# spaceandtimefdn/blitzar

Hardware: NVIDIA H100
Metric: MSM throughput (scalar*point terms/sec), ristretto255, n=2^20 per GPU (higher is better)
Workload: dtype u32 limbs (integer modular arithmetic)

## Files before the change

### blitzar_b200/api.py

```python
import ctypes as C
import os

import numpy as np

_HERE = os.path.dirname(os.path.abspath(__file__))
LIB_PATH = os.path.join(_HERE, "lib", "libblitzar_b200.so")

SXT_CPU_BACKEND, SXT_GPU_BACKEND = 1, 2
SXT_CURVE_RISTRETTO255, SXT_CURVE_BLS_381, SXT_CURVE_BN_254, SXT_CURVE_GRUMPKIN = 0, 1, 2, 3
CURVE_SIZES = {0: (160, 160, 32), 1: (144, 104, 48), 2: (96, 72, 72), 3: (96, 72, 72)}
COMPACT_BYTES = {0: 120, 1: 96, 2: 64, 3: 64}

SXT_SYMBOLS = [
    "sxt_init", "sxt_curve25519_compute_pedersen_commitments",
    "sxt_curve25519_compute_pedersen_commitments_with_generators",
    "sxt_bls12_381_g1_compute_pedersen_commitments_with_generators",
    "sxt_bn254_g1_uncompressed_compute_pedersen_commitments_with_generators",
    "sxt_grumpkin_uncompressed_compute_pedersen_commitments_with_generators",
    "sxt_ristretto255_get_generators", "sxt_curve25519_get_one_commit",
    "sxt_curve25519_prove_inner_product", "sxt_curve25519_verify_inner_product",
    "sxt_multiexp_handle_new", "sxt_multiexp_handle_new_from_file",
    "sxt_multiexp_handle_write_to_file", "sxt_multiexp_handle_free",
    "sxt_fixed_multiexponentiation", "sxt_fixed_packed_multiexponentiation",
    "sxt_fixed_vlen_multiexponentiation", "sxt_prove_sumcheck",
]
B200_SYMBOLS = [
    "b200_set_device", "b200_launch_count", "b200_point_bytes", "b200_malloc", "b200_free",
    "b200_memcpy_h2d", "b200_memcpy_d2h", "b200_synchronize", "b200_event_create",
    "b200_event_record", "b200_event_elapsed_ms", "b200_event_destroy", "b200_commit_device",
    "b200_combine_partials_device", "b200_fixed_msm_device",
    "b200_combine_partials_projective_device", "b200_set_tuning", "b200_profile_accumulate",
    "b200_profile_read", "b200_set_reduce_groups", "b200_stream",
    "b200_synthetic_generators_device", "b200_commit_host_partials",
    "b200_fixed_msm_host_partials", "b200_multiexp_handle_new_device",
    "b200_selftest_lane_arithmetic", "b200_selftest_sort", "b200_partition_table_device",
    "b200_multiexp_handle_write_partition_table",
    "b200_compute_pedersen_commitments_with_offsets", "b200_commit_device_with_offsets",
    "b200_multiexp_handle_add_partition_table", "b200_multiexp_handle_partition_window",
]


class sxt_config(C.Structure):
    _fields_ = [("backend", C.c_int), ("num_precomputed_generators", C.c_uint64)]


class sxt_sequence_descriptor(C.Structure):
    _fields_ = [("element_nbytes", C.c_uint8), ("n", C.c_uint64), ("data", C.c_void_p),
                ("is_signed", C.c_int)]


_lib = None


def lib():
    global _lib
    if _lib is None:
        if not os.path.exists(LIB_PATH):
            raise RuntimeError(f"{LIB_PATH} is missing: run `python -m blitzar_b200.build` "
                               "(blitzar_b200 has no CPU fallback)")
        L = C.CDLL(LIB_PATH)
        L.sxt_init.restype = C.c_int
        L.sxt_ristretto255_get_generators.restype = C.c_int
        L.sxt_curve25519_get_one_commit.restype = C.c_int
        L.sxt_multiexp_handle_new.restype = C.c_void_p
        L.sxt_multiexp_handle_new_from_file.restype = C.c_void_p
        L.b200_launch_count.restype = C.c_ulonglong
        L.b200_point_bytes.restype = C.c_uint
        L.b200_malloc.restype = C.c_void_p
        L.b200_multiexp_handle_new_device.restype = C.c_void_p
        L.b200_event_create.restype = C.c_void_p
        L.b200_stream.restype = C.c_void_p
        L.b200_event_elapsed_ms.restype = C.c_float
        _lib = L
    return _lib


_initialized = False


def sxt_init(backend=SXT_GPU_BACKEND, num_precomputed_generators=0, device=None):
    global _initialized
    if _initialized:
        return 0
    if device is not None:
        lib().b200_set_device(C.c_int(device))
    cfg = sxt_config(backend, num_precomputed_generators)
    rc = lib().sxt_init(C.byref(cfg))
    if rc == 0:
        _initialized = True
    return rc

# ... 170 lines not shown
    def record(self):
        lib().b200_event_record(C.c_void_p(self.e))

    def elapsed_ms(self, stop):
        return float(lib().b200_event_elapsed_ms(C.c_void_p(self.e), C.c_void_p(stop.e)))


def commit_device(curve_id, columns_shape, scalar_ptrs, generators_ptr, out_commit_ptr=None,
                  out_partial_ptr=None, offset_generators=0):
    num = len(columns_shape)
    arr = (sxt_sequence_descriptor * max(1, num))()
    for i, (n, nbytes, is_signed) in enumerate(columns_shape):
        arr[i].element_nbytes = nbytes
        arr[i].n = n
        arr[i].data = scalar_ptrs[i]
        arr[i].is_signed = int(is_signed)
    lib().b200_commit_device(C.c_uint(curve_id), C.c_void_p(out_commit_ptr),
                             C.c_void_p(out_partial_ptr), C.c_uint32(num), arr,
                             C.c_void_p(generators_ptr), C.c_uint64(offset_generators))


def commit_device_with_offsets(curve_id, columns_shape, scalar_ptrs, generators_ptr, offsets,
                               out_commit_ptr=None, out_partial_ptr=None):
    num = len(columns_shape)
    arr = (sxt_sequence_descriptor * max(1, num))()
    for i, (n, nbytes, is_signed) in enumerate(columns_shape):
        arr[i].element_nbytes = nbytes
        arr[i].n = n
        arr[i].data = scalar_ptrs[i]
        arr[i].is_signed = int(is_signed)
    offsets = _offsets(offsets, num)
    lib().b200_commit_device_with_offsets(C.c_uint(curve_id), C.c_void_p(out_commit_ptr),
                                          C.c_void_p(out_partial_ptr), C.c_uint32(num), arr,
                                          C.c_void_p(generators_ptr), _ptr(offsets))


def selftest_lane_arithmetic(warps=64, seed=1):
    lib().b200_selftest_lane_arithmetic.restype = C.c_uint
    return int(lib().b200_selftest_lane_arithmetic(C.c_uint(warps), C.c_uint(seed)))


def selftest_sort(columns_shape, scalar_ptrs, window_bits=0):
    num = len(columns_shape)
    arr = (sxt_sequence_descriptor * max(1, num))()
    for i, (n, nbytes, is_signed) in enumerate(columns_shape):
        arr[i].element_nbytes = nbytes
        arr[i].n = n
        arr[i].data = scalar_ptrs[i]
        arr[i].is_signed = int(is_signed)
    lib().b200_selftest_sort.restype = C.c_uint
    return int(lib().b200_selftest_sort(arr, C.c_uint(num), C.c_uint(window_bits)))


def synthetic_generators_device(curve_id, out_ptr, n, first=0, projective=False):
    lib().b200_synthetic_generators_device(C.c_uint(curve_id), C.c_void_p(out_ptr), C.c_uint64(n),
                                           C.c_uint64(first), C.c_int(1 if projective else 0))


def partition_table_bytes(curve_id, n, window_width):
    return -(-n // window_width) * (COMPACT_BYTES[curve_id] << window_width)


def partition_table_device(curve_id, out_ptr, gens_ptr, n, window_width=0):
    lib().b200_partition_table_device(C.c_uint(curve_id), C.c_void_p(out_ptr), C.c_void_p(gens_ptr),
                                      C.c_uint64(n), C.c_uint(window_width))


def synthetic_generators(curve_id, n, first=0, projective=False):
    stride = CURVE_SIZES[curve_id][0 if (projective or curve_id == 0) else 1]
    buf = DeviceBuffer(n * stride)
    synthetic_generators_device(curve_id, buf.ptr, n, first, projective)
    out = buf.to_host((n, stride))
    buf.free()
    return out


def commit_host_partials(curve_id, columns, generators, out_partial_ptr, offset_generators=0):
    desc, keep = make_descriptors(columns)
    lib().b200_commit_host_partials(C.c_uint(curve_id), C.c_void_p(out_partial_ptr),
                                    C.c_uint32(len(columns)), desc, _ptr(generators),
                                    C.c_uint64(offset_generators))


def fixed_msm_device(handle, out_res_ptr, out_partial_ptr, element_num_bytes, num_outputs, n,
                     scalars_ptr):
    lib().b200_fixed_msm_device(C.c_void_p(out_res_ptr), C.c_void_p(out_partial_ptr),
                                C.c_void_p(handle.h), C.c_int(0), C.c_uint(element_num_bytes),
                                None, None, C.c_uint(num_outputs), C.c_uint(n),
                                C.c_void_p(scalars_ptr))


def fixed_msm_host_partials(handle, out_partial_ptr, element_num_bytes, num_outputs, n, scalars):
    lib().b200_fixed_msm_host_partials(C.c_void_p(out_partial_ptr), C.c_void_p(handle.h),
                                       C.c_int(0), C.c_uint(element_num_bytes), None, None,
                                       C.c_uint(num_outputs), C.c_uint(n), _ptr(scalars))


def combine_partials_projective_device(curve_id, out_ptr, partials_ptr, num_parts, count):
    lib().b200_combine_partials_projective_device(C.c_uint(curve_id), C.c_void_p(out_ptr),
                                                  C.c_void_p(partials_ptr), C.c_uint32(num_parts),
                                                  C.c_uint32(count))


def synchronize():
    lib().b200_synchronize()

# ... 63 lines not shown
```

### blitzar_b200/csrc/api.cu

```cuda
#include <algorithm>
#include <cctype>
#include <cstdint>
#include <cstdio>
#include <cstdlib>
#include <cstring>
#include <condition_variable>
#include <functional>
#include <mutex>
#include <thread>
#include <memory>
#include <string>
#include <vector>

#include "engine_api.cuh"

using namespace b200;

namespace {

struct State {
  bool initialized = false;
  int device = -1;
  cudaStream_t stream = nullptr;
  cudaStream_t copy_stream = nullptr;
// ... 1296 lines not shown
    }
    if (i >= 1) {
      const int k = (int)((i - 1) & 1);
      B200_CUDA(cudaEventSynchronize(copied[k]));
      B200_REQUIRE(std::fwrite(host[k], chunk_size(i - 1), 1, f) == 1, "short write");
    }
  }
  B200_REQUIRE(std::fclose(f) == 0, "short write");
  stream_sync(s);
  for (int k = 0; k < 2; ++k) {
    if (host[k])
      B200_CUDA(cudaFreeHost(host[k]));
    B200_CUDA(cudaEventDestroy(built[k]));
    B200_CUDA(cudaEventDestroy(copied[k]));
  }
}
unsigned b200_multiexp_handle_add_partition_table(struct sxt_multiexp_handle* handle,
                                                  unsigned window_width) {
  std::lock_guard<std::mutex> lock(g_mutex);
  require_init("b200_multiexp_handle_add_partition_table");
  HandleSet* hs = reinterpret_cast<HandleSet*>(handle);
  B200_REQUIRE(hs != nullptr, "null handle");
  return handle_add_partition_table(hs, window_width);
}
unsigned b200_multiexp_handle_partition_window(const struct sxt_multiexp_handle* handle) {
  std::lock_guard<std::mutex> lock(g_mutex);
  const HandleSet* hs = reinterpret_cast<const HandleSet*>(handle);
  B200_REQUIRE(hs != nullptr, "null handle");
  return hs->shards.empty() ? 0u : hs->shards[0]->ptable_w;
}
unsigned b200_selftest_lane_arithmetic(unsigned warps, unsigned seed) {
  std::lock_guard<std::mutex> lock(g_mutex);
  require_init("b200_selftest_lane_arithmetic");
  return selftest_lane_arithmetic(ctx(), warps, seed);
}
unsigned b200_selftest_sort(const sxt_sequence_descriptor* columns, unsigned num,
                            unsigned window_bits) {
  std::lock_guard<std::mutex> lock(g_mutex);
  require_init("b200_selftest_sort");
  B200_REQUIRE(num == 0 || columns != nullptr, "columns == nullptr");
  B200_REQUIRE(window_bits <= 20, "window_bits in 0..20");
  return selftest_sort(ctx(), columns, num, window_bits);
}
void b200_set_reduce_groups(unsigned g1, unsigned gn) {
  std::lock_guard<std::mutex> lock(g_mutex);
  auto pow2 = [](unsigned v, unsigned dflt) {
    if (v < 2)
      return dflt;
    unsigned p = 2;
    while (p * 2 <= v)
      p *= 2;
    return p;
  };
  g_state.opt.reduce_g1 = pow2(g1, 16u);
  g_state.opt.reduce_gn = pow2(gn, 4u);
}
void b200_profile_accumulate(int enable) {
  std::lock_guard<std::mutex> lock(g_mutex);
  KernelTimer::get().enabled = enable != 0;
}
void b200_profile_read(float* total_ms, unsigned* launches) {
  std::lock_guard<std::mutex> lock(g_mutex);
  KernelTimer::get().read(total_ms, launches);
}
void b200_set_tuning(unsigned window_bits, unsigned chunk1, unsigned chunkn) {
  std::lock_guard<std::mutex> lock(g_mutex);
  g_state.opt.window_bits = window_bits;
  g_state.opt.chunk1 = chunk1;
  g_state.opt.chunkn = chunkn ? chunkn : 8;
}

}
```

### blitzar_b200/csrc/engine.cuh

```cuda
#pragma once
#include <cstdint>
#include <vector>

#include "engine_api.cuh"
#include "msm.cuh"
#include "partition_msm.cuh"
#include "ptable.cuh"
#include "synth.cuh"

namespace b200 {

inline uint64_t check_descriptors(const sxt_sequence_descriptor* d, uint32_t num) {
  B200_REQUIRE(d != nullptr, "descriptors == nullptr");
  uint64_t longest = 0;
  for (uint32_t i = 0; i < num; ++i) {
    B200_REQUIRE(d[i].n == 0 || d[i].data != nullptr, "descriptor.n > 0 with data == nullptr");
    B200_REQUIRE(d[i].element_nbytes != 0 && d[i].element_nbytes <= 32,
                 "descriptor.element_nbytes must be in 1..32");
    if (d[i].is_signed)
      B200_REQUIRE(d[i].element_nbytes <= 16 &&
                       (d[i].element_nbytes & (d[i].element_nbytes - 1)) == 0,
                   "signed columns need a power-of-two element_nbytes <= 16");
    B200_REQUIRE(d[i].n < (1ull << 31), "column too long");
    longest = longest < d[i].n ? d[i].n : longest;
// ... 364 lines not shown
        cost_t += (double)col.n * (col.bit_width / table_c + 1) + 2.5 * nb_t;
        cost_v += (double)(col.bit_width / cv + 1) * ((double)col.n + 2.5 * nb_v);
      }
    return cost_t < cost_v;
  }
  static std::vector<u32> partition_route(const EngineCtx& ctx, const Handle* h,
                                          const std::vector<ColumnDesc>& cols) {
    std::vector<u32> routed;
    if (!h->ptable || ctx.partition_policy == 2)
      return routed;
    const double kLookup = 1.0, kDouble = 300.0;
    const bool table_mode = prefer_table(cols, h->window_bits, h->windows, ctx.opt);
    u64 max_n = 0;
    u32 max_width = 1, ncols = 0;
    for (auto& col : cols)
      if (col.n) {
        max_n = std::max<u64>(max_n, col.n);
        max_width = std::max(max_width, col.bit_width);
        ++ncols;
      }
    if (ncols == 0)
      return routed;
    const u32 cv = ctx.opt.window_bits ? ctx.opt.window_bits
                                       : choose_window_bits(max_n, max_width, ncols, sizeof(Point));
    const double nb_v = (double)(1u << (cv - 1)), w = h->ptable_w;
    for (u32 j = 0; j < (u32)cols.size(); ++j) {
      const ColumnDesc& col = cols[j];
      if (col.n == 0)
        continue;
      const double n = col.n, b = col.bit_width;
      const double engine =
          table_mode ? n * (double)(col.bit_width / h->window_bits + 1) +
                           2.5 * (double)(1u << (h->window_bits - 1))
                     : (double)(col.bit_width / cv + 1) * (n + 2.5 * nb_v);
      const double table = kLookup * b * std::ceil(n / w) + kDouble * b;
      if (ctx.partition_policy == 1 || table < engine)
        routed.push_back(j);
    }
    return routed;
  }
  static void synth_generators(const EngineCtx& ctx, void* out_dev, uint64_t n, uint64_t first,
                               bool projective) {
    Synth<C>::generators(ctx.s, out_dev, n, first, projective);
  }
  static void partition_table(const EngineCtx& ctx, const void* gens, uint64_t n, unsigned w,
                              uint64_t first_group, uint64_t groups, void* out_dev) {
    build_partition_table<C>(ctx.s, (const Gen*)gens, n, w, first_group, groups,
                             (unsigned char*)out_dev);
  }
  static void partition_gens(const EngineCtx& ctx, const void* gens, uint64_t n, unsigned w,
                             uint64_t first_group, uint64_t groups, void* out_gens) {
    build_partition_table<C>(ctx.s, (const Gen*)gens, n, w, first_group, groups, (Gen*)out_gens);
  }
};

#define B200_DEFINE_CURVE_VTABLE(NAME, C)                                                          \
  const CurveVTable NAME = {C::kCurveId,                                                           \
                            (unsigned)sizeof(typename C::Point),                                   \
                            (unsigned)sizeof(typename C::Gen),                                     \
                            (unsigned)C::kAbiGenBytes,                                             \
                            (unsigned)C::kAbiProjBytes,                                            \
                            (unsigned)C::kAbiCommitBytes,                                          \
                            &CurveOps<C>::commit_device,                                           \
                            &CurveOps<C>::commit_device_offsets,                                   \
                            &CurveOps<C>::fixed_device,                                            \
                            &CurveOps<C>::ingest_projective,                                       \
                            &CurveOps<C>::gens_to_projective,                                      \
                            &CurveOps<C>::store,                                                   \
                            &CurveOps<C>::sum_parts,                                               \
                            &CurveOps<C>::synth_generators,                                        \
                            (unsigned)C::kAbiCompactBytes,                                         \
                            &CurveOps<C>::ingest_compact_table,                                    \
                            &CurveOps<C>::build_table,                                             \
                            &CurveOps<C>::partition_table,                                         \
                            &CurveOps<C>::partition_gens}

}
```

### blitzar_b200/csrc/engine_api.cuh

```cuda
#pragma once
#include <algorithm>
#include <cmath>
#include <cstdint>
#include <vector>

#include "../../include/blitzar_b200.h"
#include "runtime.cuh"

namespace b200 {

struct MsmOptions {
  u32 window_bits = 0;
  u32 chunk1 = 0;
  u32 chunkn = 8;
  u32 reduce_g1 = 16;
  u32 reduce_gn = 4;
  u64 quad_threshold = 32768;
  u64 max_group_entries = 1ull << 30;
  u64 max_range_entries = 1ull << 31;
  int pair_levels = -1;
  u32 pair_batch = 0;
  int range_skew = 0;
  u32 uniform_add = 2;
  u32 gens_normalized = 0;
  const u32* unit_veto = nullptr;
  u32 normalize_gens = 1;
  u32 lane_tail = 1;
  u32 scatter_window_major = 0;
  u32 sort_path = 1;
  u32 table_policy = 0;
};

struct EngineCtx {
  stream_t s;
  MsmOptions opt;
  const void* builtin;
  uint64_t num_builtin;
  stream_t tail = stream_t();
  u32 builtin_window_bits = 0, builtin_windows = 0;
  u32 partition_policy = 0;
};

struct Handle {
  unsigned curve_id;
  unsigned n;
  void* gens;
  unsigned window_bits = 0, windows = 1;
  void* ptable = nullptr;
  unsigned ptable_w = 0;
  uint64_t ptable_groups = 0;
};

inline unsigned table_window_bits(uint64_t n, size_t gen_bytes, double budget_bytes) {
  if (n < 1024)
    return 0;
  unsigned best = 0;
  double best_cost = 1e300;
  for (unsigned c = 10; c <= 20; ++c) {
    const double W = 256 / c + 1;
    if (W * (double)n * (double)gen_bytes > budget_bytes || W * (double)n >= 2147483648.0)
      continue;
    const double cost = W * (double)n + 2.5 * (double)(1u << (c - 1));
    if (cost < best_cost) {
      best_cost = cost;
      best = c;
    }
  }
  return best;
// ... 69 lines not shown
      if (n_[j] > b)
        iv.push_back({base[j] + b, base[j] + std::min(e, n_[j])});
    std::sort(iv.begin(), iv.end());
    std::vector<Piece> out;
    size_t k = 0;
    for (auto& v : iv) {
      while (segments[k].pos + segments[k].count <= v.first)
        ++k;
      const Piece& s = segments[k];
      if (!out.empty() && out.back().pos + out.back().count >= v.first && out.back().pos >= s.pos) {
        out.back().count = std::max(out.back().count, v.second - out.back().pos);
        continue;
      }
      out.push_back({s.src + (v.first - s.pos), v.first, v.second - v.first});
    }
    return out;
  }

private:
  std::vector<uint64_t> n_;
  static uint64_t offset(const uint64_t* offsets, uint32_t j) { return offsets ? offsets[j] : 0; }
};

struct CurveVTable {
  unsigned curve_id, point_bytes, gen_bytes, abi_gen_bytes, abi_proj_bytes, abi_commit_bytes;
  void (*commit_device)(const EngineCtx&, void* out_commitments, void* out_partials, uint32_t num,
                        const sxt_sequence_descriptor* d, const void* generators_dev,
                        uint64_t offset_generators, uint32_t num_ranges, range_wait_fn wait,
                        void* wait_user);
  void (*commit_device_offsets)(const EngineCtx&, void* out_commitments, void* out_partials,
                                uint32_t num, const sxt_sequence_descriptor* d,
                                const void* generators_dev, const uint64_t* offsets, bool packed,
                                uint32_t num_ranges, range_wait_fn wait, void* wait_user);
  void (*fixed_device)(const EngineCtx&, void* out_res, void* out_partials, const Handle* h,
                       int mode, unsigned element_num_bytes, const unsigned* bit_table,
                       const unsigned* lengths, unsigned num_outputs, unsigned n,
                       const uint8_t* scalars_dev);
  void (*ingest_projective)(const EngineCtx&, const void* raw_dev, void* gens, uint64_t n);
  void (*gens_to_projective)(const EngineCtx&, const void* gens, void* out_dev, uint64_t n);
  void (*store)(const EngineCtx&, const void* pts, void* out_dev, uint64_t count, bool commit);
  void (*sum_parts)(const EngineCtx&, const void* parts, uint32_t nparts, uint32_t count,
                    void* out_pts);
  void (*synth_generators)(const EngineCtx&, void* out_dev, uint64_t n, uint64_t first,
                           bool projective);
  unsigned abi_compact_bytes;
  void (*ingest_compact_table)(const EngineCtx&, const void* table_dev, unsigned window_width,
                               void* gens, uint64_t n);
  void (*build_table)(const EngineCtx&, void* table, uint64_t n, unsigned window_bits,
                      unsigned windows);
  void (*partition_table)(const EngineCtx&, const void* gens, uint64_t n, unsigned w,
                          uint64_t first_group, uint64_t groups, void* out_dev);
  void (*partition_gens)(const EngineCtx&, const void* gens, uint64_t n, unsigned w,
                         uint64_t first_group, uint64_t groups, void* out_gens);
};
extern const CurveVTable kVTableEd25519, kVTableBls12381, kVTableBn254, kVTableGrumpkin;

inline const CurveVTable& curve_vtable(unsigned curve_id) {
  switch (curve_id) {
  case SXT_CURVE_RISTRETTO255:
    return kVTableEd25519;
  case SXT_CURVE_BLS_381:
    return kVTableBls12381;
  case SXT_CURVE_BN_254:
    return kVTableBn254;
  case SXT_CURVE_GRUMPKIN:
    return kVTableGrumpkin;
  default:
    die("unsupported curve id", __FILE__, __LINE__);
  }
}

void ipa_prove(const EngineCtx& ctx, uint8_t* l_vector, uint8_t* r_vector, uint8_t* ap_value,
               uint8_t* transcript203, uint64_t n, uint64_t generators_offset,
               const uint8_t* a_vector, const uint8_t* b_vector);
int ipa_verify(const EngineCtx& ctx, uint8_t* transcript203, uint64_t n,
               uint64_t generators_offset, const uint8_t* b_vector, const uint8_t* product,
               const uint8_t* a_commit160, const uint8_t* l_vector, const uint8_t* r_vector,
               const uint8_t* ap_value);

unsigned selftest_lane_arithmetic(const EngineCtx& ctx, unsigned warps, unsigned seed);
unsigned selftest_sort(const EngineCtx& ctx, const sxt_sequence_descriptor* d, unsigned num,
                       unsigned window_bits);

void launch_builtin_generators(const EngineCtx& ctx, void* gens, uint64_t first, uint64_t n);

}
```

### blitzar_b200/csrc/msm.cuh

```cuda
#pragma once
#include <algorithm>
#include <vector>

#include "batch_affine.cuh"
#include "curve.cuh"
#include "engine_api.cuh"
#include "lanefield.cuh"

namespace b200 {

struct ColumnDesc {
  const unsigned char* base;
  u64 row_stride;
  u32 bit_offset;
  u32 bit_width;
  u32 n;
  u32 is_signed;
  u32 first_window;
  u32 num_windows;
  u32 table_n;
  u32 gen_base;
};
B200_HD u32 bucket_windows(const ColumnDesc& col) { return col.table_n ? (col.num_windows ? 1u : 0u) : col.num_windows; }

// ... 690 lines not shown
            out_pieces[2 * t] = acc;
          }
          first_seg = false;
          cur = k;
          fetch(acc, i, true);
        }
      }
    }
    if (final_level) {
      put_bucket(cur, acc, writer);
      return;
    }
    if (!writer)
      return;
    if (first_seg) {
      out_keys[2 * t] = cur;
      out_pieces[2 * t] = acc;
      out_keys[2 * t + 1] = cur;
      out_pieces[2 * t + 1] = C::identity();
    } else {
      out_keys[2 * t + 1] = cur;
      out_pieces[2 * t + 1] = acc;
    }
  }
};

struct WindowUsedBody {
  static constexpr int kBlock = 64;
  const u32* bucket_end;
  u32 nbuckets;
  u32* window_used;
  B200_HD void operator()(u64 w) const {
    u32 lo = w ? bucket_end[w * nbuckets - 1] : 0u;
    u32 hi = bucket_end[(w + 1) * nbuckets - 1];
    if (hi != lo)
      window_used[w] = 1u;
  }
};

struct WindowUsedFromCountsBody {
  static constexpr int kBlock = 128;
  const u32* counts;
  u64 nkeys;
  u32 nbuckets;
  u32* window_used;
  B200_HD void operator()(u64 t) const {
    const u64 b = t * 256, e = b + 256 < nkeys ? b + 256 : nkeys;
    for (u64 k = b; k < e; ++k)
      if (counts[k])
        window_used[k / nbuckets] = 1u;
  }
};

template <class C, class Ex = SeqExec> struct ReduceBody {
  static constexpr int kBlock = 64;
  typedef typename C::Point Point;
  const Point* X;
  const Point* Cin;
  u32 m_in, g, log2g;
  Point* Xout;
  Point* Cout;
  const u32* window_used;
  u32 nbuckets;
  B200_HD void operator()(u64 tid) const {
    const u64 t = tid / Ex::kLanes;
    const bool writer = (tid % Ex::kLanes) == 0;
    const u32 m_out = m_in / g;
    const u32 w = (u32)(t / m_out), k = (u32)(t % m_out);
    if (window_used[w] == 0) {
      if (writer) {
        Xout[t] = C::identity();
        Cout[t] = C::identity();
      }
      return;
    }
    const Point* x = X + (u64)w * m_in + (u64)k * g;
    Point run = x[g - 1];
    Point acc = Cin ? C::identity() : run;
    if (Cin) {
      acc = run;
      if (g == 1)
        acc = C::identity();
    }
    for (u32 r = g - 1; r-- > 0;) {
      C::template add<Ex>(run, run, x[r]);
      if (r > 0 || !Cin)
        C::template add<Ex>(acc, acc, run);
    }
    if (Cin) {
      const Point* cin = Cin + (u64)w * m_in + (u64)k * g;
      for (u32 r = 0; r < g; ++r)
        C::template add<Ex>(acc, acc, cin[r]);
    }
    for (u32 i = 0; i < log2g; ++i)
      C::template dbl<Ex>(run, run);
    if (writer) {
      Xout[t] = run;
      Cout[t] = acc;
    }
  }
};

template <class C, class X = SeqExec> struct CombineBody {
  static constexpr int kBlock = 32;
  typedef typename C::Point Point;
  const Point* S;
  const ColumnDesc* cols;
  u32 c;
  Point* out;
  B200_HD void operator()(u64 tid) const {
    const u64 j = tid / X::kLanes;
    const bool writer = (tid % X::kLanes) == 0;
    const ColumnDesc col = cols[j];
    if (col.num_windows == 0 || col.n == 0) {
      if (writer)
        out[j] = C::identity();
      return;
    }
    const u32 nw = bucket_windows(col);
    Point acc = S[col.first_window + nw - 1];
    for (u32 w = nw - 1; w-- > 0;) {
      for (u32 i = 0; i < c; ++i)
        C::template dbl<X>(acc, acc);
      C::template add<X>(acc, acc, S[col.first_window + w]);
    }
    if (writer)
      out[j] = acc;
  }
};

#if defined(__CUDACC__) && !defined(B200_EMULATE)
#define B200_LANE_TAIL 1
struct CombineLaneBody {
  static constexpr int kBlock = 32;
  typedef Ed25519 C;
  const C::Point* S;
  const ColumnDesc* cols;
  u32 c;
  C::Point* out;
  __device__ void operator()(u64 tid) const {
    const u64 j = tid >> 5;
    const ColumnDesc col = cols[j];
    if (col.num_windows == 0 || col.n == 0) {
      if ((tid & 31u) == 0)
        out[j] = C::identity();
      return;
    }
    const lane10::Lane L = lane10::lane_info();
    const u32 nw = bucket_windows(col);
    C::Point acc = S[col.first_window + nw - 1];
    for (u32 w = nw - 1; w-- > 0;) {
      u32 t;
      const u32 v = lane10::dbl_n(L, lane10::slice_point(L, acc), (int)c, t);
      lane10::gather_point(acc, v, t);
// ... 646 lines not shown
                          u32* d_window_used, const MsmOptions& opt, stream_t tail,
                          RangeHook* hook = nullptr) {
  const StagedRange r(s, plan, begin, end);
  if (r.total_terms == 0)
    return;
  gens += begin;
  StageRange nvtx_sort("msm: digit count + scan + scatter");
  const u64 max_entries = r.max_entries, nkeys = plan.nkeys;
  u32 L = 0;
  if constexpr (C::kBatchAffine) {
    const double mean = (double)max_entries / (double)nkeys;
    if (opt.pair_levels >= 0)
      L = (u32)opt.pair_levels;
    else if (max_entries >= (1ull << 23))
      while (L < 6 && (double)(32u << L) <= mean)
        ++L;
    while (L > 0 && max_entries + nkeys * ((1ull << L) - 1) >= (1ull << 32) - (1ull << L))
      --L;
  }
  const SortedLayout sorted = sort_entries(s, plan, r, L, opt, d_window_used);
  B200_LOG(3, "range [%llu, %llu): %llu terms, %llu entries max, c=%u, %llu keys, pair levels %u",
           (unsigned long long)begin, (unsigned long long)end, (unsigned long long)r.total_terms,
           (unsigned long long)max_entries, plan.c, (unsigned long long)nkeys, L);
  WalkInput<C> walk{gens, sorted.entries, sorted.d_m, max_entries};
  std::vector<void*> to_free;
  if (hook)
    hook->before_accumulate();
  KernelTimer::get().begin(s);
  StageRange nvtx_acc("msm: bucket accumulation");
  if constexpr (C::kBatchAffine) {
    if (L) {
      walk = run_pair_levels<C>(s, L, sorted.entries, gens, sorted.d_m, sorted.slots_max,
                                opt.pair_batch);
      to_free = {(void*)walk.gens, (void*)walk.entries};
    }
  }
  typedef typename C::Point Point;
  Point* target = add_into ? (Point*)dev_alloc(nkeys * sizeof(Point), s) : d_buckets;
  const bool unit = walk.gens == gens && opt.gens_normalized;
  const stream_t cs =
      chunk_walk<C>(s, tail, walk, sorted.d_m, unit, opt.unit_veto, target, opt, to_free);
  if (add_into) {
    launch(MergeBucketsBody<C>{sorted.counts, sorted.starts, target, d_buckets}, nkeys, cs);
    dev_free(target, cs);
  }
  to_free.insert(to_free.end(), {sorted.d_m, sorted.counts, sorted.starts});
  for (void* ptr : to_free)
    dev_free(ptr, cs);
  dev_free(sorted.entries, s);
  dev_free((void*)r.d_cols, s);
}

template <class C>
void msm_finish(stream_t s, const MsmPlan& plan, const typename C::Point* d_buckets,
                const u32* d_window_used, typename C::Point* out, const MsmOptions& opt) {
  typedef typename C::Point Point;
  StageRange nvtx_fin("msm: bucket reduction + window combination");
  const u32 total_windows = plan.total_windows, nbuckets = plan.nbuckets, ncols = plan.ncols;
  ColumnDesc* d_cols =
      (ColumnDesc*)stage_to_device(s, plan.cols.data(), ncols * sizeof(ColumnDesc));
  Point* d_S = nullptr;
  u32 m = nbuckets;
  const Point* X = d_buckets;
  const Point* Cin = nullptr;
  std::vector<void*> to_free;
  if (m == 1) {
    d_S = (Point*)dev_alloc(total_windows * sizeof(Point), s);
    copy_d2d(d_S, d_buckets, total_windows * sizeof(Point), s);
  }
  bool first = true;
  while (m > 1) {
    u32 g = first ? std::min<u32>(opt.reduce_g1, m) : std::min<u32>(opt.reduce_gn, m);
    u32 log2g = 0;
    while ((1u << log2g) < g)
      ++log2g;
    u32 m_out = m / g;
    Point* Xout = (Point*)dev_alloc((u64)total_windows * m_out * sizeof(Point), s);
    Point* Cout = (Point*)dev_alloc((u64)total_windows * m_out * sizeof(Point), s);
    if ((u64)total_windows * m_out <= opt.quad_threshold)
      launch(ReduceBody<C, QuadExecConv>{X, Cin, m, g, log2g, Xout, Cout, d_window_used, nbuckets},
             (u64)total_windows * m_out * QuadExec::kLanes, s);
    else
      launch(ReduceBody<C>{X, Cin, m, g, log2g, Xout, Cout, d_window_used, nbuckets},
             (u64)total_windows * m_out, s);
    to_free.push_back(Xout);
    if (m_out > 1)
      to_free.push_back(Cout);
    X = Xout;
    Cin = Cout;
    m = m_out;
    first = false;
    if (m == 1)
      d_S = Cout;
  }
  for (void* ptr : to_free)
    dev_free(ptr, s);
  bool uniform_windows = true;
  for (u32 j = 1; j < ncols; ++j)
    uniform_windows = uniform_windows && bucket_windows(plan.cols[j]) == bucket_windows(plan.cols[0]);
#ifdef B200_LANE_TAIL
  bool lane_done = false;
  if constexpr (C::kCurveId == kRistretto255) {
    if (ncols <= 2048 && opt.lane_tail) {
      launch(CombineLaneBody{d_S, d_cols, plan.c, out}, (u64)ncols * 32, s);
      lane_done = true;
    }
  }
  if (lane_done) {
  } else
#endif
  if (ncols <= opt.quad_threshold && uniform_windows)
    launch(CombineBody<C, QuadExecConv>{d_S, d_cols, plan.c, out}, (u64)ncols * QuadExec::kLanes,
           s);
  else if (ncols <= opt.quad_threshold)
    launch(CombineBody<C, QuadExec>{d_S, d_cols, plan.c, out}, (u64)ncols * QuadExec::kLanes, s);
  else
    launch(CombineBody<C>{d_S, d_cols, plan.c, out}, ncols, s);
  dev_free(d_S, s);
  dev_free(d_cols, s);
}

template <class C>
void msm_run(stream_t s, const typename C::Gen* gens, std::vector<ColumnDesc> cols,
             typename C::Point* out, const MsmOptions& opt = MsmOptions(), u32 num_ranges = 1,
             RangeHook* hook = nullptr, stream_t tail = stream_t()) {
  typedef typename C::Point Point;
  if (cols.empty())
    return;
  MsmPlan plan = msm_make_plan(std::move(cols), opt, sizeof(Point));
  B200_LOG(2, "msm: curve %u, %u columns, longest %llu, %llu terms, window %u bits, %u bucket sets%s",
           C::kCurveId, plan.ncols, (unsigned long long)plan.max_n,
           (unsigned long long)plan.total_terms, plan.c, plan.total_windows,
           plan.ncols && plan.cols[0].table_n ? " (fixed-base table)" : "");
  if (plan.total_terms == 0 || plan.total_windows == 0) {
    if (hook)
      hook->before_range(0, plan.max_n);
    fill_identity<C>(s, out, plan.ncols);
    return;
  }
  Point* d_buckets = (Point*)dev_alloc(plan.nkeys * sizeof(Point), s);
  fill_identity<C>(s, d_buckets, plan.nkeys);
  u32* d_window_used = (u32*)dev_alloc(plan.total_windows * sizeof(u32), s);
  dev_zero(d_window_used, plan.total_windows * sizeof(u32), s);
  if (num_ranges < 1)
    num_ranges = 1;
  const u64 limit = opt.max_range_entries ? opt.max_range_entries : (1ull << 31);
  const u64 needed = (plan.total_entries + limit - 1) / limit;
  if (needed > num_ranges)
    num_ranges = (u32)std::min<u64>(needed, plan.max_n);
// ... 18 lines not shown
```

### include/blitzar_b200.h

```cpp
#ifndef BLITZAR_B200_H
#define BLITZAR_B200_H

#include <stdint.h>

#ifdef __cplusplus
extern "C" {
#endif

#define SXT_CPU_BACKEND 1
#define SXT_GPU_BACKEND 2
#define SXT_CURVE_RISTRETTO255 0
#define SXT_CURVE_BLS_381 1
#define SXT_CURVE_BN_254 2
#define SXT_CURVE_GRUMPKIN 3
#define SXT_FIELD_SCALAR255 0
#define SXT_FIELD_GRUMPKIN 1

struct sxt_config { int backend; uint64_t num_precomputed_generators; };
struct sxt_ristretto255_compressed { uint8_t ristretto_bytes[32]; };
struct sxt_bls12_381_g1_compressed { uint8_t g1_bytes[48]; };
struct sxt_curve25519_scalar { uint8_t bytes[32]; };
struct sxt_transcript { uint8_t bytes[203]; };
struct sxt_ristretto255 { uint64_t X[5]; uint64_t Y[5]; uint64_t Z[5]; uint64_t T[5]; };
struct sxt_bls12_381_g1 { uint64_t X[6]; uint64_t Y[6]; };
// ... 94 lines not shown
void* b200_stream(void);
void* b200_event_create(void);
void b200_event_record(void* event);
float b200_event_elapsed_ms(void* start, void* stop);
void b200_event_destroy(void* event);

void b200_commit_device(unsigned curve_id, void* out_commitments, void* out_partials,
                        uint32_t num_sequences, const struct sxt_sequence_descriptor* descriptors,
                        const void* generators, uint64_t offset_generators);
void b200_commit_host_partials(unsigned curve_id, void* out_partials, uint32_t num_sequences,
                               const struct sxt_sequence_descriptor* descriptors,
                               const void* generators, uint64_t offset_generators);
void b200_compute_pedersen_commitments_with_offsets(unsigned curve_id, void* commitments,
                                                    uint32_t num_sequences,
                                                    const struct sxt_sequence_descriptor* descriptors,
                                                    const void* generators, const uint64_t* offsets);
void b200_commit_device_with_offsets(unsigned curve_id, void* out_commitments, void* out_partials,
                                     uint32_t num_sequences,
                                     const struct sxt_sequence_descriptor* descriptors,
                                     const void* generators, const uint64_t* offsets);
void b200_fixed_msm_host_partials(void* out_partials, const struct sxt_multiexp_handle* handle,
                                  int mode, unsigned element_num_bytes,
                                  const unsigned* output_bit_table, const unsigned* output_lengths,
                                  unsigned num_outputs, unsigned n, const uint8_t* scalars);
struct sxt_multiexp_handle* b200_multiexp_handle_new_device(unsigned curve_id,
                                                            const void* generators_dev,
                                                            unsigned n);
void b200_combine_partials_device(unsigned curve_id, void* out_commitments, const void* partials,
                                  uint32_t num_parts, uint32_t count);
void b200_fixed_msm_device(void* out_res, void* out_partials,
                           const struct sxt_multiexp_handle* handle, int mode,
                           unsigned element_num_bytes, const unsigned* output_bit_table,
                           const unsigned* output_lengths, unsigned num_outputs, unsigned n,
                           const uint8_t* scalars);
void b200_combine_partials_projective_device(unsigned curve_id, void* out_res,
                                             const void* partials, uint32_t num_parts,
                                             uint32_t count);
void b200_synthetic_generators_device(unsigned curve_id, void* out_generators, uint64_t n,
                                      uint64_t first, int projective);
void b200_partition_table_device(unsigned curve_id, void* out_table_dev, const void* generators_dev,
                                 uint64_t n, unsigned window_width);
void b200_multiexp_handle_write_partition_table(const struct sxt_multiexp_handle* handle,
                                                const char* filename, unsigned window_width);
unsigned b200_multiexp_handle_add_partition_table(struct sxt_multiexp_handle* handle,
                                                  unsigned window_width);
unsigned b200_multiexp_handle_partition_window(const struct sxt_multiexp_handle* handle);
unsigned b200_selftest_lane_arithmetic(unsigned warps, unsigned seed);
unsigned b200_selftest_sort(const struct sxt_sequence_descriptor* columns, unsigned num,
                            unsigned window_bits);
void b200_profile_accumulate(int enable);
void b200_profile_read(float* total_ms, unsigned* launches);
void b200_set_tuning(unsigned window_bits, unsigned chunk1, unsigned chunkn);
void b200_set_reduce_groups(unsigned g1, unsigned gn);

#ifdef __cplusplus
}
#endif
#endif
```

Before: 336.3 million.

## Replace multi-level bucket reduction with segment pass plus block-level shared-memory fold

Bucket reduction used to run as a chain of global-memory levels, each with a fixed group size. It now runs as an adaptive first segment pass, then a ReduceFoldBody kernel that folds many segment partials per block in shared memory with a tree of adds and doublings. The goal is fewer kernel launches and global round trips, plus better occupancy, during the reduction stage. A selftest compares the new path against the old one. The default reduce_g1 changes to 0 so the segment length is picked automatically.

Result: no change. 338.4 million (median of 6 runs) (+0.6%).

```diff
diff --git a/blitzar_b200/api.py b/blitzar_b200/api.py
--- a/blitzar_b200/api.py
+++ b/blitzar_b200/api.py
@@ -37,6 +37,7 @@
     "b200_multiexp_handle_write_partition_table",
     "b200_compute_pedersen_commitments_with_offsets", "b200_commit_device_with_offsets",
     "b200_multiexp_handle_add_partition_table", "b200_multiexp_handle_partition_window",
+    "b200_selftest_reduce",
 ]
 
 
@@ -313,6 +314,12 @@
     return int(lib().b200_selftest_sort(arr, C.c_uint(num), C.c_uint(window_bits)))
 
 
+def selftest_reduce(curve_id, window_bits, sets, seed=0):
+    lib().b200_selftest_reduce.restype = C.c_uint
+    return int(lib().b200_selftest_reduce(C.c_uint(curve_id), C.c_uint(window_bits), C.c_uint(sets),
+                                          C.c_uint(seed)))
+
+
 def synthetic_generators_device(curve_id, out_ptr, n, first=0, projective=False):
     lib().b200_synthetic_generators_device(C.c_uint(curve_id), C.c_void_p(out_ptr), C.c_uint64(n),
                                            C.c_uint64(first), C.c_int(1 if projective else 0))
diff --git a/blitzar_b200/csrc/api.cu b/blitzar_b200/csrc/api.cu
--- a/blitzar_b200/csrc/api.cu
+++ b/blitzar_b200/csrc/api.cu
@@ -1372,8 +1372,16 @@
       p *= 2;
     return p;
   };
-  g_state.opt.reduce_g1 = pow2(g1, 16u);
+  g_state.opt.reduce_g1 = pow2(g1, 0u);
   g_state.opt.reduce_gn = pow2(gn, 4u);
+}
+unsigned b200_selftest_reduce(unsigned curve_id, unsigned window_bits, unsigned sets,
+                              unsigned seed) {
+  std::lock_guard<std::mutex> lock(g_mutex);
+  require_init("b200_selftest_reduce");
+  B200_REQUIRE(window_bits >= 1 && window_bits <= 20, "window_bits in 1..20");
+  B200_REQUIRE(sets >= 1 && sets <= 4096, "sets in 1..4096");
+  return curve_vtable(curve_id).selftest_reduce(ctx(), window_bits, sets, seed);
 }
 void b200_profile_accumulate(int enable) {
   std::lock_guard<std::mutex> lock(g_mutex);
diff --git a/blitzar_b200/csrc/engine.cuh b/blitzar_b200/csrc/engine.cuh
--- a/blitzar_b200/csrc/engine.cuh
+++ b/blitzar_b200/csrc/engine.cuh
@@ -440,6 +440,10 @@
                              uint64_t first_group, uint64_t groups, void* out_gens) {
     build_partition_table<C>(ctx.s, (const Gen*)gens, n, w, first_group, groups, (Gen*)out_gens);
   }
+  static unsigned selftest_reduce(const EngineCtx& ctx, unsigned window_bits, unsigned sets,
+                                  unsigned seed) {
+    return reduce_selftest<C>(ctx.s, window_bits, sets, seed, ctx.opt);
+  }
 };
 
 #define B200_DEFINE_CURVE_VTABLE(NAME, C)                                                          \
@@ -461,6 +465,7 @@
                             &CurveOps<C>::ingest_compact_table,                                    \
                             &CurveOps<C>::build_table,                                             \
                             &CurveOps<C>::partition_table,                                         \
-                            &CurveOps<C>::partition_gens}
+                            &CurveOps<C>::partition_gens,                                          \
+                            &CurveOps<C>::selftest_reduce}
 
 }
diff --git a/blitzar_b200/csrc/engine_api.cuh b/blitzar_b200/csrc/engine_api.cuh
--- a/blitzar_b200/csrc/engine_api.cuh
+++ b/blitzar_b200/csrc/engine_api.cuh
@@ -13,7 +13,7 @@
   u32 window_bits = 0;
   u32 chunk1 = 0;
   u32 chunkn = 8;
-  u32 reduce_g1 = 16;
+  u32 reduce_g1 = 0;
   u32 reduce_gn = 4;
   u64 quad_threshold = 32768;
   u64 max_group_entries = 1ull << 30;
@@ -189,6 +189,7 @@
                           uint64_t first_group, uint64_t groups, void* out_dev);
   void (*partition_gens)(const EngineCtx&, const void* gens, uint64_t n, unsigned w,
                          uint64_t first_group, uint64_t groups, void* out_gens);
+  unsigned (*selftest_reduce)(const EngineCtx&, unsigned window_bits, unsigned sets, unsigned seed);
 };
 extern const CurveVTable kVTableEd25519, kVTableBls12381, kVTableBn254, kVTableGrumpkin;
 
diff --git a/blitzar_b200/csrc/msm.cuh b/blitzar_b200/csrc/msm.cuh
--- a/blitzar_b200/csrc/msm.cuh
+++ b/blitzar_b200/csrc/msm.cuh
@@ -766,6 +766,25 @@
   }
 };
 
+template <class C, class Ex>
+B200_HD void reduce_group(typename C::Point& run, typename C::Point& acc, const typename C::Point* x,
+                          const typename C::Point* cin, u32 g, u32 log2g) {
+  run = x[g - 1];
+  acc = run;
+  if (cin && g == 1)
+    acc = C::identity();
+  for (u32 r = g - 1; r-- > 0;) {
+    C::template add<Ex>(run, run, x[r]);
+    if (r > 0 || !cin)
+      C::template add<Ex>(acc, acc, run);
+  }
+  if (cin)
+    for (u32 r = 0; r < g; ++r)
+      C::template add<Ex>(acc, acc, cin[r]);
+  for (u32 i = 0; i < log2g; ++i)
+    C::template dbl<Ex>(run, run);
+}
+
 template <class C, class Ex = SeqExec> struct ReduceBody {
   static constexpr int kBlock = 64;
   typedef typename C::Point Point;
@@ -775,7 +794,6 @@
   Point* Xout;
   Point* Cout;
   const u32* window_used;
-  u32 nbuckets;
   B200_HD void operator()(u64 tid) const {
     const u64 t = tid / Ex::kLanes;
     const bool writer = (tid % Ex::kLanes) == 0;
@@ -788,32 +806,76 @@
       }
       return;
     }
-    const Point* x = X + (u64)w * m_in + (u64)k * g;
-    Point run = x[g - 1];
-    Point acc = Cin ? C::identity() : run;
-    if (Cin) {
-      acc = run;
-      if (g == 1)
-        acc = C::identity();
-    }
-    for (u32 r = g - 1; r-- > 0;) {
-      C::template add<Ex>(run, run, x[r]);
-      if (r > 0 || !Cin)
-        C::template add<Ex>(acc, acc, run);
-    }
-    if (Cin) {
-      const Point* cin = Cin + (u64)w * m_in + (u64)k * g;
-      for (u32 r = 0; r < g; ++r)
-        C::template add<Ex>(acc, acc, cin[r]);
-    }
-    for (u32 i = 0; i < log2g; ++i)
-      C::template dbl<Ex>(run, run);
+    const u64 first = (u64)w * m_in + (u64)k * g;
+    Point run, acc;
+    reduce_group<C, Ex>(run, acc, X + first, Cin ? Cin + first : nullptr, g, log2g);
     if (writer) {
       Xout[t] = run;
       Cout[t] = acc;
     }
   }
 };
+
+#ifndef B200_EMULATE
+template <class C> struct ReduceFoldBody {
+  static constexpr int kBlock = 128;
+  static constexpr u32 kQuads = kBlock / QuadExec::kLanes;
+  typedef typename C::Point Point;
+  const Point* X;
+  const Point* Cin;
+  u32 m_in, P;
+  Point* Xout;
+  Point* Cout;
+  const u32* window_used;
+  static constexpr size_t smem_bytes() { return 2 * kQuads * sizeof(Point); }
+  __device__ void run(u64 b, unsigned char* smem) const {
+    const u32 w = (u32)(b / (m_in / P));
+    if (window_used[w] == 0) {
+      if (threadIdx.x == 0) {
+        if (Xout)
+          Xout[b] = C::identity();
+        Cout[b] = C::identity();
+      }
+      return;
+    }
+    Point* sx = (Point*)smem;
+    Point* sc = sx + kQuads;
+    const u32 nq = P < kQuads ? P : kQuads, g = P / nq, log2g = 31 - __clz(g);
+    const u32 Q = threadIdx.x / QuadExec::kLanes, q = Q & (nq - 1);
+    const bool writer = (threadIdx.x % QuadExec::kLanes) == 0;
+    const u64 first = b * P + (u64)q * g;
+    Point x, c;
+    reduce_group<C, QuadExecConv>(x, c, X + first, Cin + first, g, log2g);
+    if (writer && Q < nq) {
+      sx[q] = x;
+      sc[q] = c;
+    }
+    __syncthreads();
+    for (u32 half = nq / 2; half >= 1; half /= 2) {
+      const u32 i = Q & (half - 1);
+      if (threadIdx.x / 32 * (32 / QuadExec::kLanes) < half) {
+        C::template add<QuadExecConv>(c, sc[2 * i], sc[2 * i + 1]);
+        C::template add<QuadExecConv>(c, c, sx[2 * i + 1]);
+        if (half > 1 || Xout) {
+          C::template add<QuadExecConv>(x, sx[2 * i], sx[2 * i + 1]);
+          C::template dbl<QuadExecConv>(x, x);
+        }
+      }
+      __syncthreads();
+      if (writer && Q < half) {
+        sx[i] = x;
+        sc[i] = c;
+      }
+      __syncthreads();
+    }
+    if (threadIdx.x == 0) {
+      if (Xout)
+        Xout[b] = sx[0];
+      Cout[b] = sc[0];
+    }
+  }
+};
+#endif
 
 template <class C, class X = SeqExec> struct CombineBody {
   static constexpr int kBlock = 32;
@@ -1566,37 +1628,32 @@
 }
 
 template <class C>
-void msm_finish(stream_t s, const MsmPlan& plan, const typename C::Point* d_buckets,
-                const u32* d_window_used, typename C::Point* out, const MsmOptions& opt) {
+typename C::Point* reduce_levels(stream_t s, const typename C::Point* buckets, const u32* window_used,
+                                 u32 sets, u32 nbuckets, u32 g1, u32 gn, u64 quad_threshold) {
   typedef typename C::Point Point;
-  StageRange nvtx_fin("msm: bucket reduction + window combination");
-  const u32 total_windows = plan.total_windows, nbuckets = plan.nbuckets, ncols = plan.ncols;
-  ColumnDesc* d_cols =
-      (ColumnDesc*)stage_to_device(s, plan.cols.data(), ncols * sizeof(ColumnDesc));
   Point* d_S = nullptr;
   u32 m = nbuckets;
-  const Point* X = d_buckets;
+  const Point* X = buckets;
   const Point* Cin = nullptr;
   std::vector<void*> to_free;
   if (m == 1) {
-    d_S = (Point*)dev_alloc(total_windows * sizeof(Point), s);
-    copy_d2d(d_S, d_buckets, total_windows * sizeof(Point), s);
+    d_S = (Point*)dev_alloc(sets * sizeof(Point), s);
+    copy_d2d(d_S, buckets, sets * sizeof(Point), s);
   }
   bool first = true;
   while (m > 1) {
-    u32 g = first ? std::min<u32>(opt.reduce_g1, m) : std::min<u32>(opt.reduce_gn, m);
+    u32 g = first ? std::min<u32>(g1, m) : std::min<u32>(gn, m);
     u32 log2g = 0;
     while ((1u << log2g) < g)
       ++log2g;
     u32 m_out = m / g;
-    Point* Xout = (Point*)dev_alloc((u64)total_windows * m_out * sizeof(Point), s);
-    Point* Cout = (Point*)dev_alloc((u64)total_windows * m_out * sizeof(Point), s);
-    if ((u64)total_windows * m_out <= opt.quad_threshold)
-      launch(ReduceBody<C, QuadExecConv>{X, Cin, m, g, log2g, Xout, Cout, d_window_used, nbuckets},
-             (u64)total_windows * m_out * QuadExec::kLanes, s);
+    Point* Xout = (Point*)dev_alloc((u64)sets * m_out * sizeof(Point), s);
+    Point* Cout = (Point*)dev_alloc((u64)sets * m_out * sizeof(Point), s);
+    if ((u64)sets * m_out <= quad_threshold)
+      launch(ReduceBody<C, QuadExecConv>{X, Cin, m, g, log2g, Xout, Cout, window_used},
+             (u64)sets * m_out * QuadExec::kLanes, s);
     else
-      launch(ReduceBody<C>{X, Cin, m, g, log2g, Xout, Cout, d_window_used, nbuckets},
-             (u64)total_windows * m_out, s);
+      launch(ReduceBody<C>{X, Cin, m, g, log2g, Xout, Cout, window_used}, (u64)sets * m_out, s);
     to_free.push_back(Xout);
     if (m_out > 1)
       to_free.push_back(Cout);
@@ -1609,6 +1666,156 @@
   }
   for (void* ptr : to_free)
     dev_free(ptr, s);
+  return d_S;
+}
+
+inline u32 reduce_segment_length(u64 sets, u32 nbuckets, u64 quad_threshold) {
+  u32 L = std::min<u32>(4, nbuckets);
+  while (2 * L <= std::min<u32>(32, nbuckets) && sets * (nbuckets / (2 * L)) > quad_threshold)
+    L *= 2;
+  return L;
+}
+
+#ifndef B200_EMULATE
+template <class C>
+typename C::Point* reduce_buckets(stream_t s, const typename C::Point* buckets, const u32* window_used,
+                                  u32 sets, u32 nbuckets, const MsmOptions& opt) {
+  typedef typename C::Point Point;
+  if (nbuckets == 1)
+    return reduce_levels<C>(s, buckets, window_used, sets, 1, 1, 1, 0);
+  const u32 L = opt.reduce_g1 ? std::min(opt.reduce_g1, nbuckets)
+                              : reduce_segment_length(sets, nbuckets, opt.quad_threshold);
+  u32 m = nbuckets / L;
+  const u64 pairs = (u64)sets * m;
+  Point* X = (Point*)dev_alloc(pairs * sizeof(Point), s);
+  Point* Cp = (Point*)dev_alloc(pairs * sizeof(Point), s);
+  const u32 log2L = 31 - __builtin_clz(L);
+  if (pairs <= opt.quad_threshold)
+    launch(ReduceBody<C, QuadExecConv>{buckets, nullptr, nbuckets, L, log2L, X, Cp, window_used},
+           pairs * QuadExec::kLanes, s);
+  else
+    launch(ReduceBody<C>{buckets, nullptr, nbuckets, L, log2L, X, Cp, window_used}, pairs, s);
+  const u32 per_block = ReduceFoldBody<C>::kQuads * std::max(opt.reduce_gn, 1u);
+  while (m > 1) {
+    const u32 P = std::min(m, per_block), m_out = m / P;
+    Point* Xout = m_out > 1 ? (Point*)dev_alloc((u64)sets * m_out * sizeof(Point), s) : nullptr;
+    Point* Cout = (Point*)dev_alloc((u64)sets * m_out * sizeof(Point), s);
+    launch_blocks(ReduceFoldBody<C>{X, Cp, m, P, Xout, Cout, window_used}, (u64)sets * m_out,
+                  ReduceFoldBody<C>::smem_bytes(), s);
+    dev_free(X, s);
+    dev_free(Cp, s);
+    X = Xout;
+    Cp = Cout;
+    m = m_out;
+  }
+  dev_free(X, s);
+  return Cp;
+}
+#endif
+
+B200_HD u32 selftest_hash(u64 x) {
+  x ^= x >> 33;
+  x *= 0xff51afd7ed558ccdull;
+  x ^= x >> 33;
+  x *= 0xc4ceb9fe1a85ec53ull;
+  x ^= x >> 33;
+  return (u32)x;
+}
+constexpr u32 kReduceTestPool = 64;
+template <class C> struct ReduceTestPoolBody {
+  static constexpr int kBlock = 32;
+  typename C::Point* pool;
+  u32 seed;
+  B200_HD void operator()(u64 j) const {
+    typename C::Point p;
+    if constexpr (C::kCurveId == kRistretto255) {
+      C::builtin_generator(p, (u64)seed * kReduceTestPool + j);
+    } else {
+      typename C::Point base;
+      C::gen_to_point(base, C::subgroup_generator(), false);
+      const u32 k = selftest_hash((u64)seed * kReduceTestPool + j) | 1u;
+      p = C::identity();
+      for (int b = 31; b >= 0; --b) {
+        C::dbl(p, p);
+        if ((k >> b) & 1u)
+          C::add(p, p, base);
+      }
+    }
+    pool[j] = p;
+  }
+};
+template <class C> struct ReduceTestFillBody {
+  static constexpr int kBlock = 64;
+  typedef typename C::Point Point;
+  const Point* pool;
+  u32 nbuckets, seed;
+  Point* buckets;
+  u32* window_used;
+  B200_HD void operator()(u64 i) const {
+    const u32 w = (u32)(i / nbuckets), r = (u32)(i % nbuckets), kind = (w + seed) % 5;
+    const u64 salt = (u64)seed << 40;
+    if (r == 0)
+      window_used[w] = kind != 4;
+    Point p = pool[selftest_hash(salt ^ (i >> 3)) % kReduceTestPool];
+    if (selftest_hash(salt ^ (i + (1ull << 39))) & 1u)
+      C::neg(p, p);
+    bool id = false;
+    if (kind == 0)
+      id = selftest_hash(salt ^ ((i >> 4) + (1ull << 38))) % 4 == 0;
+    else if (kind == 1)
+      id = true;
+    else if (kind == 2)
+      id = r != 0;
+    else if (kind == 3)
+      id = r != nbuckets - 1;
+    buckets[i] = id ? C::identity() : p;
+  }
+};
+
+template <class C> unsigned reduce_selftest(stream_t s, u32 c, u32 sets, u32 seed, const MsmOptions& opt) {
+#ifdef B200_EMULATE
+  (void)s, (void)c, (void)sets, (void)seed, (void)opt;
+  return ~0u;
+#else
+  typedef typename C::Point Point;
+  const u32 nbuckets = 1u << (c - 1);
+  const u64 nkeys = (u64)sets * nbuckets, bytes = (u64)sets * C::kAbiCommitBytes;
+  DevBuf<Point> pool(kReduceTestPool, s), buckets(nkeys, s);
+  DevBuf<u32> used(sets, s);
+  DevBuf<unsigned char> enc(2 * bytes, s);
+  launch(ReduceTestPoolBody<C>{pool.p, seed}, kReduceTestPool, s);
+  launch(ReduceTestFillBody<C>{pool.p, nbuckets, seed, buckets.p, used.p}, nkeys, s);
+  Point* a = reduce_levels<C>(s, buckets.p, used.p, sets, nbuckets, 16, 4, opt.quad_threshold);
+  Point* b = reduce_buckets<C>(s, buckets.p, used.p, sets, nbuckets, opt);
+  launch(StoreBody<C, true>{a, enc.p}, sets, s);
+  launch(StoreBody<C, true>{b, enc.p + bytes}, sets, s);
+  std::vector<unsigned char> h(2 * bytes);
+  copy_d2h(h.data(), enc.p, 2 * bytes, s);
+  stream_sync(s);
+  dev_free(a, s);
+  dev_free(b, s);
+  unsigned bad = 0;
+  for (u32 w = 0; w < sets; ++w)
+    bad += std::memcmp(h.data() + (u64)w * C::kAbiCommitBytes,
+                       h.data() + bytes + (u64)w * C::kAbiCommitBytes, C::kAbiCommitBytes) != 0;
+  return bad;
+#endif
+}
+
+template <class C>
+void msm_finish(stream_t s, const MsmPlan& plan, const typename C::Point* d_buckets,
+                const u32* d_window_used, typename C::Point* out, const MsmOptions& opt) {
+  typedef typename C::Point Point;
+  StageRange nvtx_fin("msm: bucket reduction + window combination");
+  const u32 ncols = plan.ncols;
+  ColumnDesc* d_cols =
+      (ColumnDesc*)stage_to_device(s, plan.cols.data(), ncols * sizeof(ColumnDesc));
+#ifdef B200_EMULATE
+  Point* d_S = reduce_levels<C>(s, d_buckets, d_window_used, plan.total_windows, plan.nbuckets, 16,
+                                4, opt.quad_threshold);
+#else
+  Point* d_S = reduce_buckets<C>(s, d_buckets, d_window_used, plan.total_windows, plan.nbuckets, opt);
+#endif
   bool uniform_windows = true;
   for (u32 j = 1; j < ncols; ++j)
     uniform_windows = uniform_windows && bucket_windows(plan.cols[j]) == bucket_windows(plan.cols[0]);
diff --git a/include/blitzar_b200.h b/include/blitzar_b200.h
--- a/include/blitzar_b200.h
+++ b/include/blitzar_b200.h
@@ -170,6 +170,7 @@
 void b200_profile_read(float* total_ms, unsigned* launches);
 void b200_set_tuning(unsigned window_bits, unsigned chunk1, unsigned chunkn);
 void b200_set_reduce_groups(unsigned g1, unsigned gn);
+unsigned b200_selftest_reduce(unsigned curve_id, unsigned window_bits, unsigned sets, unsigned seed);
 
 #ifdef __cplusplus
 }
```
